# yizhiwang96/Slice3D

Measured on AMD Instinct MI355X. Metric: occupancy query-points/sec (U-Net encode + per-query decode, 256^2 x 12 slices), higher is better.
Workload: dtype f16x3

## Files before the change

### include/slice3d_hip.h

```cpp
#ifndef SLICE3D_HIP_H
#define SLICE3D_HIP_H

#include <stddef.h>
#include <stdint.h>

#ifdef __cplusplus
extern "C" {
#endif

#define S3D_VERSION 124
#define S3D_E_ARG (-1)
#define S3D_E_WORKSPACE (-2)
#define S3D_E_ROUNDS (-3)

#define S3D_N_LEVELS 5
#define S3D_D_MODEL 128
#define S3D_N_LAYERS 3
#define S3D_FFN 2048
#define S3D_N_TOKENS_MAX 13

#define S3D_PREC_F32 0
#define S3D_PREC_F16X3 1
#define S3D_PREC_F16 2
#define S3D_PREC_BF16 3

int s3d_version(void);
const char* s3d_last_error(void);


typedef struct {
    const float* w;
    const float* b;
    const float* bn[4];
// ... 153 lines not shown
int s3d_group_norm_fwd(const float* x, const float* gamma, const float* beta, const float* film, float* y,
                       float* stats, int N, int HW, int C, int groups, float eps, int silu, void* stream);
int s3d_group_norm_film_fwd(const float* x, const float* gamma, const float* beta, const float* film, long film_stride,
                            float* y, float* stats, int N, int HW, int C, int groups, float eps, int silu, void* stream);
int s3d_group_norm2_fwd(const float* x0, int c0, const float* x1, int c1, const float* gamma, const float* beta,
                        const float* film, float* y, float* stats, int N, int HW, int groups, float eps, int silu,
                        void* stream);
int s3d_qkv_attention_fwd(const float* qkv, float* out, int N, int T, int heads, int ch, int prec, void* stream);
size_t s3d_qkv_attention_ws_bytes(int N, int T, int heads, int ch);
int s3d_qkv_attention_ws_fwd(const float* qkv, float* out, int N, int T, int heads, int ch, void* ws, size_t ws_bytes,
                             void* stream);
int s3d_resample2x_fwd(const float* x, float* y, int N, int H, int W, int C, int up, void* stream);
int s3d_small_linear_fwd(const float* x, const float* w, const float* b, float* out, int N, int K, int M,
                         int silu_in, void* stream);
int s3d_timestep_embedding_fwd(const float* t, float* out, int N, int dim, float max_period, void* stream);
int s3d_add_fwd(const float* a, const float* b, float* out, long n, void* stream);
int s3d_nchw_to_nhwc_pad(const float* in, float* out, int n, int c, int h, int w, int cpad, void* stream);
int s3d_add_nchw_fwd(const float* a, const float* b, float* out, int n, int c, int h, int w, void* stream);

int s3d_conv_strided_fwd(const void* packed, const float* x, float* out, int N, int Hin, int Win, int Hout, int Wout, int cout,
                         int cin, int ks, int stride, int pad_origin, int prec, void* stream);
int s3d_conv_plan_describe(int N, int H, int W, int cout, int cin0, int cin1, int ks, int prec, int fused_gn, size_t workspace_bytes,
                           int nsplit_out_requested, int Hin, int Win, int stride, int pad_origin, char* buf, size_t buf_len);
int s3d_wide_attention_fwd(const float* qkv, float* out, int N, int T, int C, int prec, void* stream);
int s3d_image_normalize_fwd(const float* x, const float* mean, const float* std, float* y, int n, int c, int h, int w,
                            void* stream);

typedef int (*s3d_all_reduce_sum_fn)(void* user, float* device_buf, long n_floats, void* stream);
typedef struct {
    s3d_all_reduce_sum_fn all_reduce_sum;
    void* user;
    int world_size;
    float* scratch;
} S3dSyncBn;
typedef struct {
    const float* img;
    const float* img_slices;
    const float* qry;
    const float* rot;
    const float* trans;
    const float* sdf;
    void* ev_grad_ready[3];
    const S3dSyncBn* sync_bn;
} S3dTrainBatch;
size_t s3d_train_workspace_bytes(int batch, int size, long n_qry, int n_slices);
int s3d_train_fwd_bwd(const S3dUNetParams* unet, const S3dHeadParams* head, const S3dVggParams* vgg,
// ... 142 lines not shown
```

### slice3d_amd/_lib.py

```python
import ctypes as C
import os

_HERE = os.path.dirname(os.path.abspath(__file__))
LIB_PATH = os.environ.get("S3D_HIP_LIB") or os.path.join(_HERE, "csrc", "libslice3d_hip.so")

N_LEVELS = 5
N_LAYERS = 3
PREC_F32 = 0
PREC_F16X3 = 1
PREC_F16 = 2
PREC_BF16 = 3
PREC = {"f32": PREC_F32, "f16x3": PREC_F16X3, "f16": PREC_F16, "bf16": PREC_BF16}
PROF_UNET, PROF_LATENT, PROF_SAMPLE, PROF_ATTN, PROF_FFN, PROF_FFN_FINAL, PROF_VGG, PROF_SAMPLE_PYR = range(8)
PROF_NAMES = ("unet_encode", "latent_build", "sample_tokens", "attn_layer", "ffn_layer", "ffn_final", "vgg_loss",
              "sample_pyramid")

c_float_p = C.POINTER(C.c_float)


class S3dConvParams(C.Structure):
    _fields_ = [("w", C.c_void_p), ("b", C.c_void_p), ("bn", C.c_void_p * 4)]


class S3dUNetParams(C.Structure):
# ... 101 lines not shown
    "s3d_conv_packed_bytes": (_sz, [_i, _i, _i, _i]),
    "s3d_conv_pack": (_i, [_vp, _vp, _i, _i, _i, _i, _vp, _sz, _vp]),
    "s3d_conv_fwd": (_i, [_vp, _vp, _vp, _vp, _vp, _i, _i, _i, _i, _i, _i, _i, _i, _vp, _sz, _vp]),
    "s3d_group_norm_stats_floats": (_sz, [_i, _i]),
    "s3d_group_norm_table_fwd": (_i, [_vp, _i, _vp, _i, _vp, _vp, _vp, C.c_long, _vp, _vp, _i, _i, _i, _f, _vp, _vp]),
    "s3d_group_norm_partial_fwd": (_i, [_vp, _vp, _vp, _vp, C.c_long, _vp, _vp, _i, _i, _i, _f, _i, _vp]),
    "s3d_conv_gn_supported": (_i, [_i, _i, _i, _i, _i, _i, _i, _i]),
    "s3d_conv_gn_fwd": (_i, [_vp, _vp, _vp, _vp, _vp, _i, _i, _i, _i, _i, _i, _i, _i, _vp, _i, _vp, _sz, _vp, _vp]),
    "s3d_conv_finish_fwd": (_i, [_vp, _i, _i, _i, _vp]),
    "s3d_group_norm_fwd": (_i, [_vp, _vp, _vp, _vp, _vp, _vp, _i, _i, _i, _i, _f, _i, _vp]),
    "s3d_group_norm_film_fwd": (_i, [_vp, _vp, _vp, _vp, C.c_long, _vp, _vp, _i, _i, _i, _i, _f, _i, _vp]),
    "s3d_group_norm2_fwd": (_i, [_vp, _i, _vp, _i, _vp, _vp, _vp, _vp, _vp, _i, _i, _i, _f, _i, _vp]),
    "s3d_qkv_attention_fwd": (_i, [_vp, _vp, _i, _i, _i, _i, _i, _vp]),
    "s3d_qkv_attention_ws_bytes": (_sz, [_i, _i, _i, _i]),
    "s3d_qkv_attention_ws_fwd": (_i, [_vp, _vp, _i, _i, _i, _i, _vp, _sz, _vp]),
    "s3d_resample2x_fwd": (_i, [_vp, _vp, _i, _i, _i, _i, _i, _vp]),
    "s3d_small_linear_fwd": (_i, [_vp, _vp, _vp, _vp, _i, _i, _i, _i, _vp]),
    "s3d_timestep_embedding_fwd": (_i, [_vp, _vp, _i, _i, _f, _vp]),
    "s3d_add_fwd": (_i, [_vp, _vp, _vp, _l, _vp]),
    "s3d_nchw_to_nhwc_pad": (_i, [_vp, _vp, _i, _i, _i, _i, _i, _vp]),
    "s3d_add_nchw_fwd": (_i, [_vp, _vp, _vp, _i, _i, _i, _i, _vp]),
    "s3d_conv_strided_fwd": (_i, [_vp, _vp, _vp, _i, _i, _i, _i, _i, _i, _i, _i, _i, _i, _i, _vp]),
    "s3d_conv_plan_describe": (_i, [_i, _i, _i, _i, _i, _i, _i, _i, _i, _sz, _i, _i, _i, _i, _i, C.c_char_p, _sz]),
    "s3d_wide_attention_fwd": (_i, [_vp, _vp, _i, _i, _i, _i, _vp]),
    "s3d_image_normalize_fwd": (_i, [_vp, _vp, _vp, _vp, _i, _i, _i, _i, _vp]),
    "s3d_vgg_packed_bytes": (_sz, []),
    "s3d_vgg_pack": (_i, [C.POINTER(S3dVggParams), _vp, _sz, _vp]),
    "s3d_vgg_workspace_bytes": (_sz, [_i, _i]),
    "s3d_vgg_loss_fwd": (_i, [_vp, _vp, _vp, _i, _i, _vp, _vp, _sz, _vp]),
    "s3d_train_workspace_bytes": (_sz, [_i, _i, _l, _i]),
    "s3d_train_fwd_bwd": (_i, [C.POINTER(S3dUNetParams), C.POINTER(S3dHeadParams), C.POINTER(S3dVggParams),
                               C.POINTER(S3dUNetParams), C.POINTER(S3dHeadParams), C.POINTER(S3dTrainBatch),
                               _i, _i, _l, _i, _f, C.c_ulonglong, _i, _vp, _vp, _vp, _vp, _sz, _vp]),
    "s3d_train_fwd": (_i, [C.POINTER(S3dUNetParams), C.POINTER(S3dHeadParams), C.POINTER(S3dVggParams),
                           C.POINTER(S3dTrainBatch), _i, _i, _l, _i, _f, C.c_ulonglong, _i, _vp, _vp, _vp, _vp, _sz, _vp]),
    "s3d_train_bwd": (_i, [C.POINTER(S3dUNetParams), C.POINTER(S3dHeadParams), C.POINTER(S3dVggParams),
                           C.POINTER(S3dUNetParams), C.POINTER(S3dHeadParams), C.POINTER(S3dTrainBatch),
                           _i, _i, _l, _i, _f, C.c_ulonglong, _i, _vp, _vp, _f, _f, _vp, _vp, _sz, _vp]),
    "s3d_gt_train_workspace_bytes": (_sz, [_i, _i, _l, _i]),
    "s3d_gt_train_fwd_bwd": (_i, [C.POINTER(S3dVgg16BnParams), C.POINTER(S3dGtHeadParams),
                                  C.POINTER(S3dVgg16BnParams), C.POINTER(S3dGtHeadParams), C.POINTER(S3dTrainBatch),
                                  _i, _i, _l, _i, _f, C.c_ulonglong, _i, _vp, _vp, _vp, _sz, _vp]),
    "s3d_dropout_mask": (_i, [C.c_ulonglong, _i, C.c_ulonglong, _l, _f, _vp, _vp]),
    "s3d_adam_step": (_i, [_vp, _vp, _vp, _vp, _l, _f, _f, _f, _f, _i, _vp]),
    "s3d_adam_step_multi": (_i, [_vp, _vp, _vp, _i, _vp, _vp, _vp, _f, _f, _f, _f, _i, _vp]),
    "s3d_prof_enable": (_i, [_i]),
# ... 107 lines not shown
```

### slice3d_amd/csrc/api.hip

```cpp
#include <dlfcn.h>
#include <stdarg.h>
#include <string.h>

#include <vector>
#include <mutex>

#include <math.h>

#include "conv_plan.h"
#include "decode.h"
#include "train.h"
#include "ldm_ops.h"

static thread_local char g_err[512] = "";

void s3d_set_error(const char* fmt, ...) {
    va_list ap;
    va_start(ap, fmt);
    vsnprintf(g_err, sizeof(g_err), fmt, ap);
    va_end(ap);
}

extern "C" int s3d_version(void) { return S3D_VERSION; }
extern "C" const char* s3d_last_error(void) { return g_err; }
// ... 408 lines not shown
        ConvLaunch c = conv_desc(base, E.enc[i], prec, N, res, res, 3, kEncTap[i] ? S3D_ACT_NONE : S3D_ACT_RELU);
        c.nsrc = 1;
        c.src[0] = plain_src(cur, curC);
        c.splitk_ws = splitk; c.splitk_floats = S3D_SPLITK_FLOATS;
        c.out = kEncTap[i] ? tap[tap_i] : pp[flip];
        TRY(launch_conv(c, st));
        cur = c.out;
        curC = kEncCout[i];
        if (!kEncTap[i]) {
            flip ^= 1;
            continue;
        }
        if (tap_i < 4) {
            TRY(launch_bn_relu_pool(tap[tap_i], base + E.pool_scale[tap_i], base + E.pool_shift[tap_i], pool[tap_i], N,
                                    res, res, curC, st));
            cur = pool[tap_i];
            res /= 2;
        }
        ++tap_i;
    }
    return 0;
}

extern "C" int s3d_unet_encode_fwd(const void* packed, const float* img, const S3dPyramid* out,
                                   float* slices_rec, int B, int S, int ns, int prec, void* workspace,
                                   size_t workspace_bytes, void* stream) {
    hipStream_t st = (hipStream_t)stream;
    S3D_CHECK_ARG(prec == S3D_PREC_F32 || prec == S3D_PREC_F16X3 || prec == S3D_PREC_F16 || prec == S3D_PREC_BF16,
                  "unet_encode: precision mode %d", prec);
    if (prec == S3D_PREC_BF16) prec = S3D_PREC_F16;
    S3D_CHECK_ARG(packed && img && out && workspace, "unet_encode: null argument");
    S3D_CHECK_ARG(B >= 1 && S >= 16 && S % 16 == 0, "unet_encode: B=%d S=%d (S must be a multiple of 16)", B, S);
    S3D_CHECK_ARG(ns >= 1 && ns <= 12, "unet_encode: n_slices %d", ns);
    S3D_CHECK_ARG(out->n_img == B * ns && out->size == S, "unet_encode: pyramid handle mismatch");
    const UNetLayout L = unet_layout(ns);
    const UNetWs W = unet_ws(B, S, ns);
    if (workspace_bytes < W.total * sizeof(float)) {
        s3d_set_error("unet_encode: workspace %zu < %zu bytes", workspace_bytes, W.total * sizeof(float));
        return S3D_E_WORKSPACE;
    }
    const float* base = (const float*)packed;
    float* ws = (float*)workspace;

    ProfScope prof_(S3D_PROF_UNET, st);
    float* const pp[2] = {ws + W.a, ws + W.b};
    float* const tap[5] = {ws + W.x[0], ws + W.x[1], ws + W.x[2], ws + W.x[3], ws + W.x[4]};
// ... 52 lines not shown
            }
            TRY(launch_slice_table_act(ws + W.up1_pre, base + L.up1_tab, base + L.up_c1[0].scale, base + L.up_c1[0].shift,
                                       ws + W.mid, B, ns, ro, Ct, st));
        } else {
            ConvLaunch c = {};
            c.wpk16 = prec != S3D_PREC_F32 ? (const void*)(base + L.up_cc[i].w16) : nullptr;
            c.single_pass = prec == S3D_PREC_F16;
            c.N = B * ns; c.H = rp; c.W = rp; c.ks = 2; c.up2x = 1;
            c.CoutPad = Ct; c.wpk = base + L.up_cc[i].w; c.KU = L.up_cc[i].KU;
            c.scale = base + L.up_c1[i].scale; c.shift = base + L.up_c1[i].shift;
            c.act = S3D_ACT_RELU; c.out_mode = S3D_OUT_NHWC; c.cout_store = Ct; c.out_cstride = Ct;
            c.nsrc = 1;
            c.src[0] = plain_src(prev, C);
            c.pre = ws + W.pre; c.pre_bdiv = ns;
            c.pre_tab = base + L.up_tb[i];
            c.out = ws + W.mid;
            TRY(launch_conv(c, st));
        }
        {
            ConvLaunch c = conv_desc(base, L.up_c2[i], prec, B * ns, ro, ro, 3, S3D_ACT_RELU);
            c.nsrc = 1;
            c.src[0] = plain_src(ws + W.mid, Ct);
            c.out = out->level[i + 1];
            TRY(launch_conv(c, st));
        }
        prev = out->level[i + 1];
        rp = ro;
    }
    if (slices_rec) {
        ConvLaunch c = conv_desc(base, L.outc, prec, B * ns, S, S, 1, S3D_ACT_TANH);
        c.nsrc = 1;
        c.src[0] = plain_src(prev, 32);
        c.out = slices_rec;
        c.out_mode = S3D_OUT_NCHW;
        c.cout_store = 3;
        TRY(launch_conv(c, st));
    }
    return 0;
}

static const int kVggCin[14] = {3, 64, 64, 128, 128, 256, 256, 256, 256, 512, 512, 512, 512, 512};
static const int kVggCout[14] = {64, 64, 128, 128, 256, 256, 256, 256, 512, 512, 512, 512, 512, 512};
static const int kVggPoolAfter[14] = {0, 1, 0, 1, 0, 0, 0, 1, 0, 0, 0, 1, 0, 0};
static const int kVggTap[14] = {0, 1, 0, 2, 0, 3, 0, 0, 0, 4, 0, 0, 0, 5};
static const float kVggW[5] = {1.0f / 2.6f, 1.0f / 4.8f, 1.0f / 3.7f, 1.0f / 5.6f, 10.0f / 1.5f};

// ... 673 lines not shown
```

### slice3d_amd/csrc/api_ldm.inc

```

struct GenConvLayout {
    int cout_pad, KU;
    size_t w, w16, scale, shift, total;
};
static GenConvLayout gen_conv_layout(int cout, int cin0, int cin1, int ks) {
    GenConvLayout L;
    L.cout_pad = pad16(cout);
    const int taps = ks * ks;
    L.KU = taps * (pad16(cin0) + pad16(cin1)) / 16;
    size_t off = 0;
    auto take = [&](size_t n) {
        size_t o = off;
        off += (n + 3) / 4 * 4;
        return o;
    };
    L.w = take((size_t)L.cout_pad * L.KU * 16);
    L.w16 = take((size_t)L.cout_pad * L.KU * 16);
    L.scale = take(L.cout_pad);
    L.shift = take(L.cout_pad);
    L.total = off;
    return L;
}

extern "C" size_t s3d_conv_packed_bytes(int cout, int cin0, int cin1, int ks) {
// ... 51 lines not shown
    if (gn) c.gn = *gn;
    c.splits_out = splits_out;
    if (splits_out) *splits_out = 1;
    if (workspace && workspace_bytes >= sizeof(float)) {
        c.splitk_ws = (float*)workspace;
        c.splitk_floats = workspace_bytes / sizeof(float);
    }
    return 0;
}
static int conv_fwd_impl(const void* packed, const float* x0, const float* x1, const float* residual, float* out,
                         int N, int H, int W, int cout, int cin0, int cin1, int ks, int prec, void* workspace,
                         size_t workspace_bytes, void* stream, const ConvGn* gn, int* splits_out = nullptr) {
    ConvLaunch c;
    TRY(conv_fwd_desc(c, packed, x0, x1, residual, out, N, H, W, cout, cin0, cin1, ks, prec, workspace, workspace_bytes, gn, splits_out));
    return launch_conv(c, (hipStream_t)stream);
}

extern "C" int s3d_conv_fwd(const void* packed, const float* x0, const float* x1, const float* residual, float* out,
                            int N, int H, int W, int cout, int cin0, int cin1, int ks, int prec, void* workspace,
                            size_t workspace_bytes, void* stream) {
    return conv_fwd_impl(packed, x0, x1, residual, out, N, H, W, cout, cin0, cin1, ks, prec, workspace, workspace_bytes, stream,
                         nullptr);
}
extern "C" int s3d_conv_gn_supported(int cout, int cin0, int cin1, int ks, int prec, int H, int W, int has_workspace) {
    if (ks != 3 || (prec != S3D_PREC_F16X3 && prec != S3D_PREC_F16)) return 0;
    if (cout <= 0 || cin0 <= 0 || cin1 < 0 || cout % 32 || cin0 % 32 || cin1 % 32) return 0;
    if (cin0 + cin1 > S3D_GN_CMAX) return 0;
    if (H > 0 && W > 0 && conv_below_lds_tile(H, W) && !has_workspace) return 0;
    return 1;
}
extern "C" int s3d_conv_gn_fwd(const void* packed, const float* x0, const float* x1, const float* residual, float* out,
                               int N, int H, int W, int cout, int cin0, int cin1, int ks, int prec, const float* table,
                               int silu, void* workspace, size_t workspace_bytes, int* nsplit_out, void* stream) {
    S3D_CHECK_ARG(table, "conv_gn_fwd: null table");
    const ConvGn gn = {table, silu};
    return conv_fwd_impl(packed, x0, x1, residual, out, N, H, W, cout, cin0, cin1, ks, prec, workspace, workspace_bytes, stream,
                         &gn, nsplit_out);
}
static int partial_to_gn(const S3dConvPartial* p, int N, int HW, GnPartial& g) {
    S3D_CHECK_ARG(p->part && p->out && p->conv_packed && p->nsplit >= 2, "conv partial: bad descriptor");
    const GenConvLayout L = gen_conv_layout(p->cout, p->cin0, p->cin1, p->ks);
    S3D_CHECK_ARG(L.cout_pad == p->cout, "conv partial: cout %d is padded to %d", p->cout, L.cout_pad);
    g.part = p->part; g.nsplit = p->nsplit; g.shift = (const float*)p->conv_packed + L.shift; g.res = p->residual; g.fin = p->out;
    (void)N; (void)HW;
    return 0;
}
// ... 97 lines not shown
```

### slice3d_amd/csrc/api_ldm_ae.inc

```

static int conv_strided_desc(ConvLaunch& c, const void* packed, const float* x, float* out, int N, int Hin, int Win, int Hout, int Wout,
                             int cout, int cin, int ks, int stride, int pad_origin, int prec) {
    S3D_CHECK_ARG(packed && x && out && N >= 1 && Hin >= 1 && Win >= 1 && Hout >= 1 && Wout >= 1 && cin >= 1 && cout % 4 == 0,
                  "conv_strided: bad arguments");
    S3D_CHECK_ARG((ks == 1 || ks == 3) && stride >= 1 && (pad_origin == 0 || (pad_origin == 1 && ks == 3 && stride > 1)),
                  "conv_strided: ks=%d stride=%d pad_origin=%d", ks, stride, pad_origin);
    S3D_CHECK_ARG(prec == S3D_PREC_F32 || prec == S3D_PREC_F16X3, "conv_strided: precision mode %d", prec);
    const GenConvLayout L = gen_conv_layout(cout, cin, 0, ks);
    const float* b = (const float*)packed;
    c = {};
    c.N = N; c.H = Hout; c.W = Wout; c.ks = ks;
    c.stride = stride; c.Hin = Hin; c.Win = Win; c.pad_origin = pad_origin;
    c.CoutPad = L.cout_pad; c.wpk = b + L.w; c.KU = L.KU;
    const bool f16 = L.KU % 2 == 0 && cin % 32 == 0;
    c.wpk16 = (prec == S3D_PREC_F16X3 && f16) ? (const void*)(b + L.w16) : nullptr;
    c.scale = nullptr;
    c.shift = b + L.shift; c.act = S3D_ACT_NONE;
    c.out_mode = S3D_OUT_NHWC; c.cout_store = cout; c.out_cstride = cout;
    c.nsrc = 1;
    c.src[0] = plain_src(x, pad16(cin));
    c.out = out;
    return 0;
}
extern "C" int s3d_conv_strided_fwd(const void* packed, const float* x, float* out, int N, int Hin, int Win, int Hout, int Wout,
// ... 5 lines not shown

extern "C" int s3d_conv_plan_describe(int N, int H, int W, int cout, int cin0, int cin1, int ks, int prec, int fused_gn,
                                      size_t workspace_bytes, int nsplit_out_requested, int Hin, int Win, int stride, int pad_origin,
                                      char* buf, size_t buf_len) {
    S3D_CHECK_ARG(buf && buf_len > 0, "conv_plan_describe: no buffer");
    static float some[4];
    const ConvGn gn = {some, 1};
    int nsplit = 0;
    ConvLaunch c;
    if (Hin > 0 || Win > 0 || stride > 0) {
        S3D_CHECK_ARG(!fused_gn && !nsplit_out_requested && !workspace_bytes && !cin1, "conv_plan_describe: the strided entry point takes one source, no GroupNorm, no workspace");
        TRY(conv_strided_desc(c, some, some, some, N, Hin, Win, H, W, cout, cin0, ks, stride, pad_origin, prec));
    } else {
        S3D_CHECK_ARG(fused_gn || !nsplit_out_requested, "conv_plan_describe: nsplit_out is an argument of s3d_conv_gn_fwd");
        TRY(conv_fwd_desc(c, some, some, cin1 > 0 ? some : nullptr, nullptr, some, N, H, W, cout, cin0, cin1, ks, prec, some, workspace_bytes,
                          fused_gn ? &gn : nullptr, nsplit_out_requested ? &nsplit : nullptr));
    }
    const ConvPlan p = conv_plan(c, conv_tuning());
    if (p.err) return p.err;
    conv_plan_describe(c, p, buf, buf_len);
    return 0;
}

extern "C" int s3d_wide_attention_fwd(const float* qkv, float* out, int N, int T, int C, int prec, void* stream) {
    S3D_CHECK_ARG(qkv && out, "wide_attention: null argument");
    S3D_CHECK_ARG(prec == S3D_PREC_F32 || prec == S3D_PREC_F16X3, "wide_attention: precision mode %d", prec);
    return launch_wide_attention(qkv, out, N, T, C, (hipStream_t)stream);
}

extern "C" int s3d_image_normalize_fwd(const float* x, const float* mean, const float* stdv, float* y, int n, int c, int h, int w,
                                       void* stream) {
    S3D_CHECK_ARG(x && mean && stdv && y, "image_normalize: null argument");
    return launch_image_normalize(x, mean, stdv, y, n, c, (long)h * w, (hipStream_t)stream);
}
```

### slice3d_amd/csrc/conv.h

```cpp
#pragma once
#include "common.h"
#include "dropout.h"

struct ConvSrc {
    const float* p;
    int C;
    int bdiv, bmod, sbcast;
};

#define S3D_GN_SLICES 64
#define S3D_GN_CMAX 1536
struct ConvGn {
    const float* table;
    int silu;
};

enum { S3D_ACT_NONE = 0, S3D_ACT_RELU = 1, S3D_ACT_TANH = 2 };
enum { S3D_OUT_NHWC = 0, S3D_OUT_CONVT = 1, S3D_OUT_NCHW = 2 };

struct ConvLaunch {
    ConvSrc src[2];
    int nsrc;
    int N, H, W;
    int ks;
// ... 7 lines not shown
    int single_pass;
    const float* scale;
    const float* shift;
    int act;
    float* out;
    int out_mode;
    int cout_store;
    int out_cstride;
    const float* residual;
    int out_accumulate;
    int xcd_remap;
    const float* gate;
    float gate_scale;
    unsigned long long drop_base;
    float* splitk_ws;
    size_t splitk_floats;
    DropCfg drop;
    ConvGn gn;
    const float* pre;
    int pre_bdiv, pre_bmod;
    int* splits_out;
    int up2x;
    const float* pre_tab;
    int tap_oy, tap_ox;
    int out_py, out_px;
};

int launch_conv(const ConvLaunch& a, hipStream_t stream);
int launch_conv_splitk_finish(const ConvLaunch& a, int nsplit, hipStream_t stream);

enum { S3D_PACK_LINEAR = 0, S3D_PACK_CONV = 1, S3D_PACK_CONVT = 2, S3D_PACK_CONV_DGRAD = 3,
       S3D_PACK_CONVT_DGRAD = 4, S3D_PACK_LINEAR_T = 5 };
struct PackArgs {
    const float* src;
    float* dst;
    int kind;
    int n_valid, n_pad;
    int KU_total, u_off, ku_seg;
    int ld, k_valid;
    int taps, cseg, cseg_valid, cin_tot, cin_begin;
    int ct;
    int f16;
    int chunk_ku;
};
int launch_pack(const PackArgs& a, hipStream_t stream);
class PackBatchScope {
// ... 39 lines not shown
```

### slice3d_amd/csrc/conv.hip

```cpp
#include <stdlib.h>
#include "conv_plan.h"
#include <utility>
#include <vector>

template <int MT, int NT>
__device__ __forceinline__ void conv_epilogue(const ConvLaunch& a, f32x4 (&acc)[MT][NT], const int (&pn)[MT],
                                              const int (&py)[MT], const int (&px)[MT], const bool (&pv)[MT],
                                              int jt0, int g) {
    const bool convt32 = a.out_mode == S3D_OUT_CONVT && a.cout_store % 32 == 0;
    if (NT % 2 == 0 && (a.out_mode == S3D_OUT_NHWC || convt32)) {
        const int m = threadIdx.x & 15;
        const bool lo = m < 8;
#pragma unroll
        for (int np = 0; np < NT / 2; ++np) {
            const int co = (jt0 + 2 * np) * 16 + 16 * (m >> 3) + 4 * g;
            const f32x4 sc = a.scale ? ld4(a.scale + co) : f32x4{1.f, 1.f, 1.f, 1.f};
            const f32x4 sh = a.shift ? ld4(a.shift + co) : zero4();
            const int ct = a.cout_store, cq = convt32 ? co / ct : 0, ccol = convt32 ? co - cq * ct : co;
            const bool col_ok = convt32 ? cq < 4 : co < a.cout_store;
#pragma unroll
            for (int mt = 0; mt < MT; ++mt) {
                f32x4 val[2];
                s3d_full_line_pair(acc[mt][2 * np], acc[mt][2 * np + 1], m, val[0], val[1]);
                const long ob = convt32 ? ((long)(pn[mt] * 2 * a.H + 2 * py[mt] + (cq >> 1)) * (2 * a.W) + 2 * px[mt] + (cq & 1)) * ct
// ... 835 lines not shown
    bool pv[MT];
#pragma unroll
    for (int mt = 0; mt < MT; ++mt) {
        pn[mt] = n;
        py[mt] = y0 + MT * wp + mt;
        px[mt] = x0 + m;
        pv[mt] = py[mt] < a.H && px[mt] < a.W;
    }
    if (gridDim.y > 1) {
        float* part = a.splitk_ws + (size_t)blockIdx.y * ((size_t)a.N * a.H * a.W * a.CoutPad);
#pragma unroll
        for (int mt = 0; mt < MT; ++mt)
            if (pv[mt]) {
                float* o = part + ((size_t)(n * a.H + py[mt]) * a.W + px[mt]) * a.CoutPad + 4 * g;
#pragma unroll
                for (int nt = 0; nt < NT; ++nt) st4(o + (jt0 + nt) * 16, acc[mt][nt]);
            }
        C3_STAMP(6);
        return;
    }
    conv_epilogue<MT, NT>(a, acc, pn, py, px, pv, jt0, g);
}

struct UpStep {
    int ey, ex, iy, ix;
};
template <int NPY, int NPX>
__host__ __device__ constexpr UpStep up_step(int s) {
    int k = 0;
    for (int ey = 0; ey <= NPY; ++ey)
        for (int ex = 0; ex <= NPX; ++ex)
            for (int iy = 0; iy < NPY; ++iy)
                for (int ix = 0; ix < NPX; ++ix)
                    if (ey - iy >= 0 && ey - iy <= 1 && ex - ix >= 0 && ex - ix <= 1) {
                        if (k == s) return UpStep{ey, ex, iy, ix};
                        ++k;
                    }
    return UpStep{-1, -1, -1, -1};
}
template <int... S, class F>
__device__ __forceinline__ void up_static_for(std::integer_sequence<int, S...>, F&& f) {
    (f(std::integral_constant<int, S>{}), ...);
}

template <int MT, int WP, int WC, int NPY, int NPX, int NBUF, int OCC>
__global__ __launch_bounds__(256, OCC) void conv_up2x_lds_f16x3_kernel(const ConvLaunch a, int tiles_x, int tiles_y) {
// ... 366 lines not shown

static_assert(kSmallHalo == C3S_HP && kSmallHalo1 == C3S_HP1, "conv_plan.h: pixels the small-map kernel parks");
static const ConvTuning g_conv_tuning = conv_tuning_from_env();
const ConvTuning& conv_tuning() { return g_conv_tuning; }

struct ConvKernel {
    ConvFamily family;
    int targ[7];
    void (*launch)(const ConvLaunch& a, const ConvPlan& p, hipStream_t stream);
};
#define CK_ARGS(...) __VA_ARGS__
#define CK(FAMILY, KERNEL, ARGS, ...)                                                                                       \
    {FAMILY, {__VA_ARGS__}, [](const ConvLaunch& a, const ConvPlan& p, hipStream_t stream) {                                 \
         hipLaunchKernelGGL((KERNEL<__VA_ARGS__>), dim3(p.grid_x, p.grid_y), dim3(p.block), 0, stream, CK_ARGS ARGS);        \
     }}
#define CK_TILE(...)                   \
    CK(CONV_IGEMM, conv_igemm_kernel, (a), __VA_ARGS__, 1, 0, 0), CK(CONV_IGEMM, conv_igemm_kernel, (a), __VA_ARGS__, 2, 0, 0),       \
    CK(CONV_IGEMM, conv_igemm_kernel, (a), __VA_ARGS__, 3, 0, 0), CK(CONV_IGEMM, conv_igemm_kernel, (a), __VA_ARGS__, 3, 1, 0),       \
    CK(CONV_IGEMM_F16X3, conv_igemm_f16x3_kernel, (a), __VA_ARGS__, 1, 0), CK(CONV_IGEMM_F16X3, conv_igemm_f16x3_kernel, (a), __VA_ARGS__, 2, 0), \
    CK(CONV_IGEMM_F16X3, conv_igemm_f16x3_kernel, (a), __VA_ARGS__, 3, 0), CK(CONV_IGEMM_F16X3, conv_igemm_f16x3_kernel, (a), __VA_ARGS__, 3, 1)
#define CK_LDS(...) CK(CONV_LDS, conv3x3_lds_f16x3_kernel, (a, p.tiles_x, p.tiles_y, p.chunks_per_split), __VA_ARGS__)
#define CK_SMALL(...) CK(CONV_SMALL, conv3x3_small_f16x3_kernel, (a, p.chunks_per_split), __VA_ARGS__)
#define CK_UP2X(...) CK(CONV_UP2X_LDS, conv_up2x_lds_f16x3_kernel, (a, p.tiles_x, p.tiles_y), __VA_ARGS__)
#define CK_STREAM(KC) CK(CONV_LIN_STREAM, lin_stream_f16x3_kernel, (a, p.n_tasks), KC)
static const ConvKernel kConvKernels[] = {
    CK_TILE(4, 4, 2, 2), CK_TILE(2, 4, 2, 2), CK_TILE(1, 4, 2, 2), CK_TILE(1, 1, 2, 2), CK_TILE(4, 4, 4, 1), CK_TILE(2, 2, 2, 2),
    CK_TILE(4, 2, 4, 1), CK_TILE(4, 1, 4, 1), CK_TILE(1, 1, 4, 1),
    CK(CONV_IGEMM, conv_igemm_kernel, (a), 1, 1, 2, 2, 2, 1, 1),
    CK_LDS(4, 2, 2, 2, 0, 0), CK_LDS(4, 2, 2, 2, 1, 0), CK_LDS(4, 2, 2, 2, 0, 1),
    CK_LDS(2, 4, 1, 2, 0, 0), CK_LDS(2, 4, 1, 2, 1, 0), CK_LDS(2, 4, 1, 2, 0, 1), CK_LDS(2, 4, 1, 1, 0, 0),
    CK_SMALL(1, 0, 9), CK_SMALL(2, 0, 9), CK_SMALL(4, 0, 9), CK_SMALL(1, 1, 9), CK_SMALL(2, 1, 9), CK_SMALL(4, 1, 9),
    CK_SMALL(1, 0, 1), CK_SMALL(2, 0, 1), CK_SMALL(4, 0, 1),
    CK_UP2X(4, 2, 2, 1, 2, 2, 2), CK_UP2X(2, 4, 1, 2, 2, 1, 2),
    CK_STREAM(1), CK_STREAM(2), CK_STREAM(3),
    {CONV_LIN_ROWS, {}, [](const ConvLaunch& a, const ConvPlan& p, hipStream_t stream) {
         hipLaunchKernelGGL(lin_rows_f16x3_kernel, dim3(p.grid_x), dim3(p.block), 0, stream, a);
     }}};

int launch_conv(const ConvLaunch& a_in, hipStream_t stream) {
    ConvLaunch a = a_in;
    a.xcd_remap = 1;
    const ConvPlan p = conv_plan(a, g_conv_tuning);
    if (p.err) return p.err;
    const ConvKernel* k = nullptr;
    for (const ConvKernel& e : kConvKernels)
        if (e.family == p.family && std::equal(e.targ, e.targ + 7, p.targ)) {
            k = &e;
            break;
        }
    S3D_CHECK_ARG(k, "conv: the plan names a kernel instantiation that is not built");
    for (int par = 0; par < (p.per_parity ? 4 : 1); ++par) {
        if (p.per_parity) {
            a.wpk = a_in.wpk + (size_t)par * (a.CoutPad / 16) * a.KU * 256;
            a.out_py = par >> 1; a.out_px = par & 1;
            a.tap_oy = a.out_py - 1; a.tap_ox = a.out_px - 1;
        }
        k->launch(a, p, stream);
        S3D_LAUNCH_CHECK();
    }
    if (a.splits_out) *a.splits_out = p.splits;
    return p.finish ? launch_conv_splitk_finish(a, p.splits, stream) : 0;
}
#undef CK_ARGS
#undef CK
#undef CK_TILE
#undef CK_LDS
#undef CK_SMALL
#undef CK_UP2X
#undef CK_STREAM

__device__ __forceinline__ void pack_frag_body(const PackArgs& a) {
    const long total = (long)(a.n_pad / 16) * a.ku_seg * 256;
    for (long idx = (long)blockIdx.x * blockDim.x + threadIdx.x; idx < total;
         idx += (long)gridDim.x * blockDim.x) {
        int e, lane, ul, j, k;
        if (!a.f16) {
            e = idx & 3; lane = (idx >> 2) & 63;
            const long fu = idx >> 8;
            ul = (int)(fu % a.ku_seg); j = (int)(fu / a.ku_seg);
            k = 16 * ul + 4 * (lane >> 4) + e;
        } else {
            const int t = idx & 7;
            lane = (idx >> 3) & 63;
            const long fu = idx >> 9;
            const int u32 = (int)(fu % (a.ku_seg / 2));
            j = (int)(fu / (a.ku_seg / 2));
            k = 32 * u32 + 8 * (lane >> 4) + t;
            ul = u32; e = t;
        }
        const int n = 16 * j + (lane & 15);
        float v = 0.f;
        if (n < a.n_valid) {
// ... 474 lines not shown
```

### slice3d_amd/csrc/conv_plan.h

```cpp
#pragma once
#include <stdlib.h>
#include <algorithm>
#include "conv.h"

struct ConvTuning {
    bool small3_on, small1_on;
    long small3_pmax, small1_pmax;
};
inline ConvTuning conv_tuning_from_env() {
    const char *e3 = getenv("S3D_CONV_SMALL"), *e1 = getenv("S3D_CONV_SMALL_1X1");
    const int v3 = e3 ? atoi(e3) : 1, v1 = e1 ? atoi(e1) : 1;
    return {v3 != 0, v1 != 0, v3 > 1 ? v3 : 32, v1 > 1 ? v1 : 64};
}
const ConvTuning& conv_tuning();

enum ConvFamily { CONV_IGEMM, CONV_IGEMM_F16X3, CONV_LIN_ROWS, CONV_LIN_STREAM, CONV_LDS, CONV_SMALL, CONV_UP2X_LDS, CONV_N_FAMILIES };
static const struct { const char* name; int nargs; const char* bools; } kConvFamily[CONV_N_FAMILIES] = {
    {"conv_igemm_kernel", 7, "0000011"},       {"conv_igemm_f16x3_kernel", 6, "000001"}, {"lin_rows_f16x3_kernel", 0, ""},
    {"lin_stream_f16x3_kernel", 1, "0"},       {"conv3x3_lds_f16x3_kernel", 6, "000011"}, {"conv3x3_small_f16x3_kernel", 3, "010"},
    {"conv_up2x_lds_f16x3_kernel", 7, "0000000"}};

struct ConvPlan {
    int err;
    ConvFamily family;
    int targ[7];
    unsigned grid_x, grid_y, block;
    int splits, chunks_per_split;
    int tiles_x, tiles_y;
    long n_tasks;
    bool finish;
    bool per_parity;
};

constexpr long kSmallHalo = 160, kSmallHalo1 = 64;
constexpr int kLinRowsTile = 192;

inline bool conv_same_grid(const ConvLaunch& a) { return !((a.Hin && a.Hin != a.H) || (a.Win && a.Win != a.W)); }
inline bool conv_chunked_sources(const ConvLaunch& a) {
    for (int s = 0; s < a.nsrc; ++s)
        if (a.src[s].C % 32 || a.src[s].sbcast) return false;
    return true;
}
inline bool conv_splittable(const ConvLaunch& a) { return a.splitk_ws && a.out_mode == S3D_OUT_NHWC; }
// ... 61 lines not shown
        S3D_CHECK_ARG(a.nsrc == 1 && !a.src[0].sbcast && a.src[0].C % 32 == 0 && a.CoutPad % 32 == 0 && a.KU == a.src[0].C / 4,
                      "conv: the composed ConvTranspose -> 3x3 takes one plain source (C %d, Cout %d, KU %d)", a.src[0].C, a.CoutPad, a.KU);
        S3D_CHECK_ARG(!a.pad_origin && a.out_cstride >= a.CoutPad && a.src[0].bdiv >= 1 && a.src[0].bmod >= 0 && a.pre_bdiv >= 1 && a.pre_bmod >= 0,
                      "conv: the composed ConvTranspose -> 3x3: pad_origin %d, channel stride %d < %d, or a bad image rule", a.pad_origin, a.out_cstride, a.CoutPad);
        S3D_CHECK_ARG(a.drop.p <= 0.f && !a.gate && !a.residual && !a.out_accumulate && (a.act == S3D_ACT_NONE || a.act == S3D_ACT_RELU),
                      "conv: the composed ConvTranspose -> 3x3 takes scale / shift / ReLU only");
        if (!a.wpk16) {
            const long nblk = ((P + 31) / 32) * (a.CoutPad / 32);
            CONV_GRID_CHECK(nblk, 1);
            p.per_parity = true;
            conv_plan_kernel(p, CONV_IGEMM, {1, 1, 2, 2, 2, 1, 1}, nblk);
            return 0;
        }
        const long nblk = tiles * (a.CoutPad / co_wg) * (co_wg == 64 ? 2 : 1);
        CONV_GRID_CHECK(nblk, 0);
        if (co_wg == 64) conv_plan_kernel(p, CONV_UP2X_LDS, {4, 2, 2, 1, 2, 2, 2}, nblk);
        else conv_plan_kernel(p, CONV_UP2X_LDS, {2, 4, 1, 2, 2, 1, 2}, nblk);
        return 0;
    }
    S3D_CHECK_ARG(!a.pre_tab, "conv: a border-class table without the composed ConvTranspose -> 3x3");
    const bool f16_chunks = a.wpk16 && a.KU % 2 == 0 && conv_chunked_sources(a);
    const bool plain = a.stride <= 1 && conv_same_grid(a);

    if (a.ks == 3 && plain && f16_chunks && a.CoutPad % 32 == 0 && (!conv_below_lds_tile(a.H, a.W) || conv_splittable(a))) {
        const long nblk = tiles * (a.CoutPad / co_wg);
        CONV_GRID_CHECK(nblk, 0);
        const long halo = (long)a.N * (a.H + 2) * (a.W + 2);
        const bool small = t.small3_on && conv_splittable(a) && co_wg == 64 && halo <= kSmallHalo &&
                           (P <= std::min(t.small3_pmax, 64L) || ((long)a.H * a.W <= 16 && P <= 64));
        const long nblk_k = small ? a.CoutPad / 64 : nblk;
        conv_plan_splits(p, a, nblk_k, conv_splittable(a) && nblk_k < 512);
        if (small && p.splits > 1) {
            conv_plan_small(p, a, P, halo, 9);
            return 0;
        }
        int ct = 0;
        for (int s = 0; s < a.nsrc; ++s) ct += a.src[s].C;
        S3D_CHECK_ARG(!a.gn.table || ct <= S3D_GN_CMAX, "conv: fused GroupNorm over %d channels", ct);
        const int nbuf = co_wg == 32 && !a.gn.table && !a.pre && p.chunks_per_split <= 2 ? 1 : 2;
        if (co_wg == 64) conv_plan_kernel(p, CONV_LDS, {4, 2, 2, 2, a.gn.table != nullptr, a.pre != nullptr}, nblk, (unsigned)p.splits);
        else conv_plan_kernel(p, CONV_LDS, {2, 4, 1, nbuf, a.gn.table != nullptr, a.pre != nullptr}, nblk, (unsigned)p.splits);
        return 0;
    }
    S3D_CHECK_ARG(!a.gn.table, "conv: a fused GroupNorm needs the LDS-staged 3x3 kernel (ks 3, stride 1, channel counts multiples of 32)");

    if (t.small1_on && a.ks == 1 && a.stride <= 1 && !a.Hin && !a.Win && f16_chunks && a.CoutPad % 64 == 0 && conv_splittable(a) &&
// ... 63 lines not shown
```

Before: 12.05 million.

## Add weight-stationary persistent 3x3 conv kernel for small-channel U-Net levels

Adds a persistent kernel that loads the full 3x3 weight slice for a 32-channel output block into LDS once and then walks many spatial tiles. Input halo loads are software-pipelined two steps ahead in registers and double-buffered in LDS. The U-Net encoder enables it for convolutions with at most 32 channels, and the planner picks it when there are enough tiles to fill the CUs. It aims to cut repeated weight reloads and launch or tail overhead on large, thin feature maps, at the cost of a fixed grid that may balance load worse, plus extra planner complexity.

```diff
diff --git a/include/slice3d_hip.h b/include/slice3d_hip.h
--- a/include/slice3d_hip.h
+++ b/include/slice3d_hip.h
@@ -8,7 +8,7 @@
 extern "C" {
 #endif
 
-#define S3D_VERSION 124
+#define S3D_VERSION 125
 #define S3D_E_ARG (-1)
 #define S3D_E_WORKSPACE (-2)
 #define S3D_E_ROUNDS (-3)
@@ -208,6 +208,11 @@
                          int cin, int ks, int stride, int pad_origin, int prec, void* stream);
 int s3d_conv_plan_describe(int N, int H, int W, int cout, int cin0, int cin1, int ks, int prec, int fused_gn, size_t workspace_bytes,
                            int nsplit_out_requested, int Hin, int Win, int stride, int pad_origin, char* buf, size_t buf_len);
+int s3d_conv_ws_fwd(const void* packed, const float* x0, const float* x1, const float* residual, float* out, int N, int H, int W,
+                    int cout, int cin0, int cin1, int ks, int prec, void* workspace, size_t workspace_bytes, void* stream,
+                    int max_workgroups, const float* scale, int relu, const float* pre, int pre_bdiv, int route, int stride);
+int s3d_conv_plan_ws_describe(int N, int H, int W, int cout, int cin0, int cin1, int ks, int prec, size_t workspace_bytes, int ws,
+                              int max_workgroups, int cus, char* buf, size_t buf_len);
 int s3d_wide_attention_fwd(const float* qkv, float* out, int N, int T, int C, int prec, void* stream);
 int s3d_image_normalize_fwd(const float* x, const float* mean, const float* std, float* y, int n, int c, int h, int w,
                             void* stream);
diff --git a/slice3d_amd/_lib.py b/slice3d_amd/_lib.py
--- a/slice3d_amd/_lib.py
+++ b/slice3d_amd/_lib.py
@@ -147,6 +147,8 @@
     "s3d_add_nchw_fwd": (_i, [_vp, _vp, _vp, _i, _i, _i, _i, _vp]),
     "s3d_conv_strided_fwd": (_i, [_vp, _vp, _vp, _i, _i, _i, _i, _i, _i, _i, _i, _i, _i, _i, _vp]),
     "s3d_conv_plan_describe": (_i, [_i, _i, _i, _i, _i, _i, _i, _i, _i, _sz, _i, _i, _i, _i, _i, C.c_char_p, _sz]),
+    "s3d_conv_ws_fwd": (_i, [_vp, _vp, _vp, _vp, _vp, _i, _i, _i, _i, _i, _i, _i, _i, _vp, _sz, _vp, _i, _vp, _i, _vp, _i, _i, _i]),
+    "s3d_conv_plan_ws_describe": (_i, [_i, _i, _i, _i, _i, _i, _i, _i, _sz, _i, _i, _i, C.c_char_p, _sz]),
     "s3d_wide_attention_fwd": (_i, [_vp, _vp, _i, _i, _i, _i, _vp]),
     "s3d_image_normalize_fwd": (_i, [_vp, _vp, _vp, _vp, _i, _i, _i, _i, _vp]),
     "s3d_vgg_packed_bytes": (_sz, []),
diff --git a/slice3d_amd/csrc/api.hip b/slice3d_amd/csrc/api.hip
--- a/slice3d_amd/csrc/api.hip
+++ b/slice3d_amd/csrc/api.hip
@@ -454,6 +454,7 @@
     return 0;
 }
 
+constexpr int kUnetWsMaxC = 32;
 extern "C" int s3d_unet_encode_fwd(const void* packed, const float* img, const S3dPyramid* out,
                                    float* slices_rec, int B, int S, int ns, int prec, void* workspace,
                                    size_t workspace_bytes, void* stream) {
@@ -552,6 +553,7 @@
             c.nsrc = 1;
             c.src[0] = plain_src(ws + W.mid, Ct);
             c.out = out->level[i + 1];
+            c.ws = Ct <= kUnetWsMaxC;
             TRY(launch_conv(c, st));
         }
         prev = out->level[i + 1];
diff --git a/slice3d_amd/csrc/api_ldm.inc b/slice3d_amd/csrc/api_ldm.inc
--- a/slice3d_amd/csrc/api_ldm.inc
+++ b/slice3d_amd/csrc/api_ldm.inc
@@ -97,6 +97,31 @@
     return conv_fwd_impl(packed, x0, x1, residual, out, N, H, W, cout, cin0, cin1, ks, prec, workspace, workspace_bytes, stream,
                          nullptr);
 }
+static int conv_ws_desc(ConvLaunch& c, const void* packed, const float* x0, const float* x1, const float* residual, float* out, int N,
+                        int H, int W, int cout, int cin0, int cin1, int ks, int prec, void* workspace, size_t workspace_bytes,
+                        int max_workgroups, const float* scale, int relu, const float* pre, int pre_bdiv, int route, int stride) {
+    TRY(conv_fwd_desc(c, packed, x0, x1, residual, out, N, H, W, cout, cin0, cin1, ks, prec, workspace, workspace_bytes, nullptr, nullptr));
+    S3D_CHECK_ARG(max_workgroups >= 0 && (!pre || pre_bdiv >= 1), "conv_ws_fwd: max_workgroups %d, pre_bdiv %d", max_workgroups, pre_bdiv);
+    c.scale = scale;
+    c.act = relu ? S3D_ACT_RELU : S3D_ACT_NONE;
+    c.pre = pre; c.pre_bdiv = pre ? pre_bdiv : 0;
+    c.ws = route ? 2 : 0;
+    c.ws_max_wg = max_workgroups;
+    S3D_CHECK_ARG(stride >= 0 && stride <= 2, "conv_ws_fwd: stride %d", stride);
+    if (stride > 1) {
+        c.stride = stride; c.Hin = stride * H; c.Win = stride * W;
+    }
+    return 0;
+}
+extern "C" int s3d_conv_ws_fwd(const void* packed, const float* x0, const float* x1, const float* residual, float* out, int N, int H,
+                               int W, int cout, int cin0, int cin1, int ks, int prec, void* workspace, size_t workspace_bytes,
+                               void* stream, int max_workgroups, const float* scale, int relu, const float* pre, int pre_bdiv, int route,
+                               int stride) {
+    ConvLaunch c;
+    TRY(conv_ws_desc(c, packed, x0, x1, residual, out, N, H, W, cout, cin0, cin1, ks, prec, workspace, workspace_bytes, max_workgroups,
+                     scale, relu, pre, pre_bdiv, route, stride));
+    return launch_conv(c, (hipStream_t)stream);
+}
 extern "C" int s3d_conv_gn_supported(int cout, int cin0, int cin1, int ks, int prec, int H, int W, int has_workspace) {
     if (ks != 3 || (prec != S3D_PREC_F16X3 && prec != S3D_PREC_F16)) return 0;
     if (cout <= 0 || cin0 <= 0 || cin1 < 0 || cout % 32 || cin0 % 32 || cin1 % 32) return 0;
diff --git a/slice3d_amd/csrc/api_ldm_ae.inc b/slice3d_amd/csrc/api_ldm_ae.inc
--- a/slice3d_amd/csrc/api_ldm_ae.inc
+++ b/slice3d_amd/csrc/api_ldm_ae.inc
@@ -51,6 +51,22 @@
     return 0;
 }
 
+extern "C" int s3d_conv_plan_ws_describe(int N, int H, int W, int cout, int cin0, int cin1, int ks, int prec, size_t workspace_bytes,
+                                         int ws, int max_workgroups, int cus, char* buf, size_t buf_len) {
+    S3D_CHECK_ARG(buf && buf_len > 0, "conv_plan_ws_describe: no buffer");
+    S3D_CHECK_ARG(ws >= 0 && ws <= 2 && cus >= 1, "conv_plan_ws_describe: ws %d, cus %d", ws, cus);
+    static float some[4];
+    ConvLaunch c;
+    TRY(conv_ws_desc(c, some, some, cin1 > 0 ? some : nullptr, nullptr, some, N, H, W, cout, cin0, cin1, ks, prec, some, workspace_bytes,
+                     max_workgroups, nullptr, 0, nullptr, 0, 0, 0));
+    c.ws = ws;
+    c.ws_cus = cus;
+    const ConvPlan p = conv_plan(c, conv_tuning());
+    if (p.err) return p.err;
+    conv_plan_describe(c, p, buf, buf_len);
+    return 0;
+}
+
 extern "C" int s3d_wide_attention_fwd(const float* qkv, float* out, int N, int T, int C, int prec, void* stream) {
     S3D_CHECK_ARG(qkv && out, "wide_attention: null argument");
     S3D_CHECK_ARG(prec == S3D_PREC_F32 || prec == S3D_PREC_F16X3, "wide_attention: precision mode %d", prec);
diff --git a/slice3d_amd/csrc/conv.h b/slice3d_amd/csrc/conv.h
--- a/slice3d_amd/csrc/conv.h
+++ b/slice3d_amd/csrc/conv.h
@@ -53,6 +53,9 @@
     int* splits_out;
     int up2x;
     const float* pre_tab;
+    int ws;
+    int ws_max_wg;
+    int ws_cus;
     int tap_oy, tap_ox;
     int out_py, out_px;
 };
diff --git a/slice3d_amd/csrc/conv.hip b/slice3d_amd/csrc/conv.hip
--- a/slice3d_amd/csrc/conv.hip
+++ b/slice3d_amd/csrc/conv.hip
@@ -1,5 +1,6 @@
 #include <stdlib.h>
 #include "conv_plan.h"
+#include <type_traits>
 #include <utility>
 #include <vector>
 
@@ -881,6 +882,191 @@
     conv_epilogue<MT, NT>(a, acc, pn, py, px, pv, jt0, g);
 }
 
+template <int HALVES, int NBUF, int NCH, bool PRE>
+__global__ __launch_bounds__(256 * HALVES) void conv3x3_ws_f16x3_kernel(const ConvLaunch a, int tiles_x, int tiles_y, long tpw) {
+    constexpr int MT = 2, NT = 2;
+    __shared__ __attribute__((aligned(16))) _Float16 s_w[NT * 9 * NCH * 1024];
+    __shared__ __attribute__((aligned(16))) _Float16 s_in[HALVES][NBUF][2][C3_HALO * C3_PXS];
+    const int tid = threadIdx.x & 255, half = threadIdx.x >> 8;
+    const int lane = tid & 63, wp = tid >> 6;
+    const int m = lane & 15, g = lane >> 4;
+    const int n_co_blk = a.CoutPad / 32;
+    const int nb = (int)gridDim.x;
+    const bool by_xcd = nb % (8 * n_co_blk) == 0;
+    const int grp = by_xcd ? (int)blockIdx.x % 8 : 0, j = by_xcd ? (int)blockIdx.x / 8 : (int)blockIdx.x;
+    const long wg_grp = (long)((by_xcd ? nb / 8 : nb) / n_co_blk) * HALVES;
+    const int blk_co = j % n_co_blk;
+    const long t_first = grp * tpw * wg_grp + (j / n_co_blk) * HALVES + half;
+    const int tiles_map = tiles_x * tiles_y;
+    const long n_task = (long)a.N * tiles_map;
+    const int KU32 = a.KU >> 1;
+    const int jt0 = blk_co * NT;
+    const int cu0 = a.src[0].C >> 5, cu1 = a.nsrc > 1 ? a.src[1].C >> 5 : 0;
+    const int nchunk = cu0 + cu1, lg = nchunk - 1;
+    if (KU32 != 9 * nchunk || nchunk > NCH || nchunk < 1) return;
+    const long n_step = ((tpw << lg) + 1) & ~1L;
+    auto live = [&](long s) { return t_first + (s >> lg) * wg_grp < n_task; };
+
+    {
+        const f32x4* wsrc = reinterpret_cast<const f32x4*>(reinterpret_cast<const _Float16*>(a.wpk16) + (size_t)jt0 * KU32 * 1024);
+        f32x4* wdst = reinterpret_cast<f32x4*>(s_w);
+        for (int i = threadIdx.x; i < NT * KU32 * 128; i += 256 * HALVES) wdst[i] = wsrc[i];
+    }
+
+    constexpr int NSLOT = C3_HALO * 8;
+    constexpr int NPRE = (NSLOT + 255) / 256;
+    f32x4 preA[NPRE], preB[NPRE];
+    unsigned okA = 0u, okB = 0u;
+    auto fetch = [&](f32x4 (&pre)[NPRE], unsigned& okm, long s) {
+        const long task = min(t_first + (s >> lg) * wg_grp, n_task - 1);
+        const int ch = (int)(s & lg);
+        const int n = (int)(task / tiles_map), tile = (int)(task - (long)n * tiles_map);
+        const int ty = tile / tiles_x, tx = tile - ty * tiles_x;
+        const int x0 = tx * 16, y0 = ty * 8;
+        const ConvSrc& S = a.src[ch < cu0 ? 0 : 1];
+        const int c = ch < cu0 ? ch : ch - cu0;
+        const int ni = (S.bmod ? n % S.bmod : n) / S.bdiv;
+        okm = 0u;
+#pragma unroll
+        for (int i = 0; i < NPRE; ++i) {
+            const int slot = tid + 256 * i;
+            const int pix = slot >> 3, q4 = slot & 7;
+            const int hy = pix / 18, hx = pix - hy * 18;
+            const int y = y0 + hy - 1, x = x0 + hx - 1;
+            const bool ok = slot < NSLOT && y >= 0 && y < a.H && x >= 0 && x < a.W;
+            const long off = ((long)(ni * a.H + (ok ? y : 0)) * a.W + (ok ? x : 0)) * S.C + 32 * c + 4 * q4;
+            pre[i] = ld4(S.p + off);
+            if (ok) okm |= 1u << i;
+        }
+    };
+    auto park = [&](const f32x4 (&pre)[NPRE], unsigned okm, int buf) {
+#pragma unroll
+        for (int i = 0; i < NPRE; ++i) {
+            const int slot = tid + 256 * i;
+            if (slot < NSLOT) {
+                const int pix = slot >> 3, q4 = slot & 7;
+                const f32x4 v = (okm >> i) & 1u ? pre[i] : zero4();
+                s3d_half4 hi, lo;
+#pragma unroll
+                for (int t = 0; t < 4; ++t) {
+                    const _Float16 h = (_Float16)v[t];
+                    hi[t] = h;
+                    lo[t] = (_Float16)(v[t] - (float)h);
+                }
+                const int po = pix * C3_PXS + C3_SWZ(pix, q4 >> 1) + 4 * (q4 & 1);
+                *reinterpret_cast<s3d_half4*>(&s_in[half][buf][0][po]) = hi;
+                *reinterpret_cast<s3d_half4*>(&s_in[half][buf][1][po]) = lo;
+            }
+        }
+    };
+
+    const int e_co = jt0 * 16 + 16 * (m >> 3) + 4 * g;
+    const bool col_ok = e_co < a.cout_store;
+    const f32x4 e_sc = a.scale ? ld4(a.scale + e_co) : f32x4{1.f, 1.f, 1.f, 1.f};
+    const f32x4 e_sh = a.shift ? ld4(a.shift + e_co) : zero4();
+    f32x4 acc[MT][NT];
+    auto body = [&](long s, const f32x4 (&nx)[NPRE], unsigned oknx, f32x4 (&fr)[NPRE], unsigned& okfr) {
+        const bool valid = live(s);
+        const long task = t_first + (s >> lg) * wg_grp;
+        const int ch = (int)(s & lg);
+        const int n = (int)(task / tiles_map), tile = (int)(task - (long)n * tiles_map);
+        const int ty = tile / tiles_x, tx = tile - ty * tiles_x;
+        const int x0 = tx * 16, y0 = ty * 8;
+        if (ch == 0) {
+#pragma unroll
+            for (int mt = 0; mt < MT; ++mt) {
+                const int y = y0 + MT * wp + mt, x = x0 + m;
+#pragma unroll
+                for (int nt = 0; nt < NT; ++nt) acc[mt][nt] = conv_acc_init<PRE>(a, valid && y < a.H && x < a.W, n, y, x, (jt0 + nt) * 16 + 4 * g);
+            }
+        }
+        fetch(fr, okfr, s + 2);
+        if (valid) {
+            const int sr = ch < cu0 ? 0 : 1, c = sr ? ch - cu0 : ch, cu = sr ? cu1 : cu0;
+            const _Float16* lw = s_w + ((sr ? 9 * cu0 : 0) + c) * 1024 + lane * 8;
+            const _Float16* sh = s_in[half][s & (NBUF - 1)][0];
+            const _Float16* sl = s_in[half][s & (NBUF - 1)][1];
+            auto taps = [&](auto single) {
+                constexpr bool SINGLE = decltype(single)::value;
+#pragma unroll
+                for (int tap = 0; tap < 9; ++tap) {
+                    const int dy = tap / 3, dx = tap % 3;
+                    s3d_half8 wh[NT], wl[NT], bh[MT], bl[MT];
+#pragma unroll
+                    for (int nt = 0; nt < NT; ++nt) {
+                        const _Float16* f = lw + (nt * KU32 + tap * cu) * 1024;
+                        wh[nt] = *reinterpret_cast<const s3d_half8*>(f);
+                        if (!SINGLE) wl[nt] = *reinterpret_cast<const s3d_half8*>(f + 512);
+                    }
+#pragma unroll
+                    for (int mt = 0; mt < MT; ++mt) {
+                        const int pix = (MT * wp + mt + dy) * 18 + m + dx;
+                        const int po = pix * C3_PXS + C3_SWZ(pix, g);
+                        bh[mt] = *reinterpret_cast<const s3d_half8*>(sh + po);
+                        if (!SINGLE) bl[mt] = *reinterpret_cast<const s3d_half8*>(sl + po);
+                    }
+#pragma unroll
+                    for (int nt = 0; nt < NT; ++nt) {
+                        if (!SINGLE) {
+#pragma unroll
+                            for (int mt = 0; mt < MT; ++mt)
+                                acc[mt][nt] = __builtin_amdgcn_mfma_f32_16x16x32_f16(wh[nt], bl[mt], acc[mt][nt], 0, 0, 0);
+#pragma unroll
+                            for (int mt = 0; mt < MT; ++mt)
+                                acc[mt][nt] = __builtin_amdgcn_mfma_f32_16x16x32_f16(wl[nt], bh[mt], acc[mt][nt], 0, 0, 0);
+                        }
+#pragma unroll
+                        for (int mt = 0; mt < MT; ++mt)
+                            acc[mt][nt] = __builtin_amdgcn_mfma_f32_16x16x32_f16(wh[nt], bh[mt], acc[mt][nt], 0, 0, 0);
+                    }
+                }
+            };
+            if (a.single_pass) taps(std::true_type{});
+            else taps(std::false_type{});
+        }
+        if (NBUF == 1) __syncthreads();
+        park(nx, oknx, (int)((s + 1) & (NBUF - 1)));
+        __syncthreads();
+        if (valid && ch == lg) {
+#pragma unroll
+            for (int mt = 0; mt < MT; ++mt) {
+                const int py = y0 + MT * wp + mt, px = x0 + m;
+                const bool pv = py < a.H && px < a.W;
+                f32x4 val[2];
+                s3d_full_line_pair(acc[mt][0], acc[mt][1], m, val[0], val[1]);
+                const long ob = ((long)(n * a.H + py) * a.W + px) * a.out_cstride;
+                const unsigned ob_lo = s3d_row_ror8_u32((unsigned)ob), ob_hi = s3d_row_ror8_u32((unsigned)((unsigned long long)ob >> 32));
+                const bool pvp = s3d_row_ror8_u32(pv ? 1u : 0u) != 0u;
+                const long obp = (long)(((unsigned long long)ob_hi << 32) | ob_lo);
+#pragma unroll
+                for (int k = 0; k < 2; ++k) {
+                    const bool own = (k == 0) == (m < 8);
+                    if (!(own ? pv : pvp) || !col_ok) continue;
+                    f32x4 v = val[k] * e_sc + e_sh;
+                    if (a.act == S3D_ACT_RELU) {
+#pragma unroll
+                        for (int i = 0; i < 4; ++i) v[i] = fmaxf(v[i], 0.f);
+                    } else if (a.act == S3D_ACT_TANH) {
+#pragma unroll
+                        for (int i = 0; i < 4; ++i) v[i] = tanhf(v[i]);
+                    }
+                    __builtin_nontemporal_store(v, reinterpret_cast<f32x4*>(a.out + (own ? ob : obp) + e_co));
+                }
+            }
+        }
+    };
+
+    fetch(preA, okA, 0);
+    fetch(preB, okB, 1);
+    park(preA, okA, 0);
+    __syncthreads();
+#pragma unroll 1
+    for (long s = 0; s < n_step; s += 2) {
+        body(s, preB, okB, preA, okA);
+        body(s + 1, preA, okA, preB, okB);
+    }
+}
+
 struct UpStep {
     int ey, ex, iy, ix;
 };
@@ -1293,6 +1479,7 @@
 #define CK_LDS(...) CK(CONV_LDS, conv3x3_lds_f16x3_kernel, (a, p.tiles_x, p.tiles_y, p.chunks_per_split), __VA_ARGS__)
 #define CK_SMALL(...) CK(CONV_SMALL, conv3x3_small_f16x3_kernel, (a, p.chunks_per_split), __VA_ARGS__)
 #define CK_UP2X(...) CK(CONV_UP2X_LDS, conv_up2x_lds_f16x3_kernel, (a, p.tiles_x, p.tiles_y), __VA_ARGS__)
+#define CK_WS(...) CK(CONV_LDS_WS, conv3x3_ws_f16x3_kernel, (a, p.tiles_x, p.tiles_y, p.n_tasks), __VA_ARGS__)
 #define CK_STREAM(KC) CK(CONV_LIN_STREAM, lin_stream_f16x3_kernel, (a, p.n_tasks), KC)
 static const ConvKernel kConvKernels[] = {
     CK_TILE(4, 4, 2, 2), CK_TILE(2, 4, 2, 2), CK_TILE(1, 4, 2, 2), CK_TILE(1, 1, 2, 2), CK_TILE(4, 4, 4, 1), CK_TILE(2, 2, 2, 2),
@@ -1303,6 +1490,7 @@
     CK_SMALL(1, 0, 9), CK_SMALL(2, 0, 9), CK_SMALL(4, 0, 9), CK_SMALL(1, 1, 9), CK_SMALL(2, 1, 9), CK_SMALL(4, 1, 9),
     CK_SMALL(1, 0, 1), CK_SMALL(2, 0, 1), CK_SMALL(4, 0, 1),
     CK_UP2X(4, 2, 2, 1, 2, 2, 2), CK_UP2X(2, 4, 1, 2, 2, 1, 2),
+    CK_WS(2, 2, 1, 0), CK_WS(2, 2, 1, 1), CK_WS(2, 1, 2, 0), CK_WS(2, 1, 2, 1),
     CK_STREAM(1), CK_STREAM(2), CK_STREAM(3),
     {CONV_LIN_ROWS, {}, [](const ConvLaunch& a, const ConvPlan& p, hipStream_t stream) {
          hipLaunchKernelGGL(lin_rows_f16x3_kernel, dim3(p.grid_x), dim3(p.block), 0, stream, a);
@@ -1311,6 +1499,7 @@
 int launch_conv(const ConvLaunch& a_in, hipStream_t stream) {
     ConvLaunch a = a_in;
     a.xcd_remap = 1;
+    if (a.ws) a.ws_cus = s3d_cu_count();
     const ConvPlan p = conv_plan(a, g_conv_tuning);
     if (p.err) return p.err;
     const ConvKernel* k = nullptr;
@@ -1339,6 +1528,7 @@
 #undef CK_SMALL
 #undef CK_UP2X
 #undef CK_STREAM
+#undef CK_WS
 
 __device__ __forceinline__ void pack_frag_body(const PackArgs& a) {
     const long total = (long)(a.n_pad / 16) * a.ku_seg * 256;
diff --git a/slice3d_amd/csrc/conv_plan.h b/slice3d_amd/csrc/conv_plan.h
--- a/slice3d_amd/csrc/conv_plan.h
+++ b/slice3d_amd/csrc/conv_plan.h
@@ -6,19 +6,20 @@
 struct ConvTuning {
     bool small3_on, small1_on;
     long small3_pmax, small1_pmax;
+    bool ws_on;
 };
 inline ConvTuning conv_tuning_from_env() {
-    const char *e3 = getenv("S3D_CONV_SMALL"), *e1 = getenv("S3D_CONV_SMALL_1X1");
+    const char *e3 = getenv("S3D_CONV_SMALL"), *e1 = getenv("S3D_CONV_SMALL_1X1"), *ew = getenv("S3D_CONV_WS");
     const int v3 = e3 ? atoi(e3) : 1, v1 = e1 ? atoi(e1) : 1;
-    return {v3 != 0, v1 != 0, v3 > 1 ? v3 : 32, v1 > 1 ? v1 : 64};
+    return {v3 != 0, v1 != 0, v3 > 1 ? v3 : 32, v1 > 1 ? v1 : 64, !ew || atoi(ew) != 0};
 }
 const ConvTuning& conv_tuning();
 
-enum ConvFamily { CONV_IGEMM, CONV_IGEMM_F16X3, CONV_LIN_ROWS, CONV_LIN_STREAM, CONV_LDS, CONV_SMALL, CONV_UP2X_LDS, CONV_N_FAMILIES };
+enum ConvFamily { CONV_IGEMM, CONV_IGEMM_F16X3, CONV_LIN_ROWS, CONV_LIN_STREAM, CONV_LDS, CONV_SMALL, CONV_UP2X_LDS, CONV_LDS_WS, CONV_N_FAMILIES };
 static const struct { const char* name; int nargs; const char* bools; } kConvFamily[CONV_N_FAMILIES] = {
     {"conv_igemm_kernel", 7, "0000011"},       {"conv_igemm_f16x3_kernel", 6, "000001"}, {"lin_rows_f16x3_kernel", 0, ""},
     {"lin_stream_f16x3_kernel", 1, "0"},       {"conv3x3_lds_f16x3_kernel", 6, "000011"}, {"conv3x3_small_f16x3_kernel", 3, "010"},
-    {"conv_up2x_lds_f16x3_kernel", 7, "0000000"}};
+    {"conv_up2x_lds_f16x3_kernel", 7, "0000000"}, {"conv3x3_ws_f16x3_kernel", 4, "0001"}};
 
 struct ConvPlan {
     int err;
@@ -126,6 +127,29 @@
     const bool f16_chunks = a.wpk16 && a.KU % 2 == 0 && conv_chunked_sources(a);
     const bool plain = a.stride <= 1 && conv_same_grid(a);
 
+    if (a.ws) {
+        int cin = 0;
+        for (int s = 0; s < a.nsrc; ++s) cin += a.src[s].C;
+        const bool ok = a.ks == 3 && plain && !a.Hin && !a.Win && f16_chunks && cin <= 64 && a.CoutPad % 32 == 0 && a.CoutPad <= 64 &&
+                        !a.splitk_ws && !a.splits_out && !a.gn.table && a.out_mode == S3D_OUT_NHWC && !conv_below_lds_tile(a.H, a.W) &&
+                        a.drop.p <= 0.f && !a.gate && !a.residual && !a.out_accumulate && tiles < (1L << 30);
+        S3D_CHECK_ARG(a.ws != 2 || ok, "conv: the weight-stationary 3x3 serves ks 3, stride 1, split precision, whole 32-channel chunks of at most 64 input "
+                      "channels, at most 64 output channels, NHWC output with scale / shift / activation only, no split-K workspace, no fused GroupNorm, maps of at least 8 x 16");
+        const int n_co = a.CoutPad / 32;
+        long wgs = a.ws_cus > 0 ? a.ws_cus : 256;
+        const bool enough = tiles * n_co >= 2 * wgs;
+        if (ok && (a.ws == 2 || (t.ws_on && enough))) {
+            if (a.ws_max_wg > 0) wgs = std::min(wgs, (long)a.ws_max_wg);
+            wgs = std::min(wgs, (tiles + 1) / 2 * n_co);
+            wgs = std::max((long)n_co, wgs - wgs % n_co);
+            const long walkers = wgs / n_co * 2;
+            p.n_tasks = (tiles + walkers - 1) / walkers;
+            if (cin == 32) conv_plan_kernel(p, CONV_LDS_WS, {2, 2, 1, a.pre != nullptr}, wgs, 1, 512);
+            else conv_plan_kernel(p, CONV_LDS_WS, {2, 1, 2, a.pre != nullptr}, wgs, 1, 512);
+            return 0;
+        }
+    }
+
     if (a.ks == 3 && plain && f16_chunks && a.CoutPad % 32 == 0 && (!conv_below_lds_tile(a.H, a.W) || conv_splittable(a))) {
         const long nblk = tiles * (a.CoutPad / co_wg);
         CONV_GRID_CHECK(nblk, 0);
```

New measurement: 12.07 million (median of 6 runs). No clear change (+0.2%).
